# UCL-CCS/Nbed

Measured on AMD Instinct MI355X. Metric: embedded_scf_cycles_per_sec, higher is better.
Workload: dtype f64

## Files before the change

### nbed_amd/csrc/elementwise.hip

```cpp
#include "nbx_common.h"
#include "jk_m4_layout.h"
#include "jk_packed.h"
#include "jk_s4_layout.h"

namespace {

constexpr int TILE = 32;
constexpr int DENS_MAX_NOCC = 64;

__global__ void final_reduce_kernel(const double* __restrict__ partial, int nblocks, int nout,
                                    double* __restrict__ out, int sqrt_from, const int* __restrict__ tail = nullptr,
                                    int tail_n = 0) {
    __shared__ double red[17];
    if ((int)threadIdx.x < tail_n) out[nout + threadIdx.x] = (double)tail[threadIdx.x];
    for (int o = 0; o < nout; ++o) {
        double t = 0.0;
        for (int b = threadIdx.x; b < nblocks; b += blockDim.x) t += partial[(int64_t)b * nout + o];
        t = nbx_block_sum(t, red);
        if (threadIdx.x == 0) out[o] = (o >= sqrt_from) ? sqrt(t) : t;
        __syncthreads();
    }
}

__device__ __forceinline__ void load_tile(const double* __restrict__ M, int N, int r0, int c0,
                                          double (*lds)[TILE + 1]) {
    for (int r = threadIdx.y; r < TILE; r += blockDim.y) {
        const int gr = r0 + r, gc = c0 + threadIdx.x;
        lds[r][threadIdx.x] = (gr < N && gc < N) ? M[(int64_t)gr * N + gc] : 0.0;
    }
}

__global__ void trace_prod_kernel(const double* __restrict__ A, const double* __restrict__ B, int N,
                                  double* __restrict__ partial) {
    __shared__ double bt[TILE][TILE + 1];
    __shared__ double red[17];
    const int b = blockIdx.z;
    const int64_t n2 = (int64_t)N * N;
    A += b * n2;
    B += b * n2;
    const int i0 = blockIdx.y * TILE, j0 = blockIdx.x * TILE;
    load_tile(B, N, j0, i0, bt);
    __syncthreads();
    double acc = 0.0;
    for (int r = threadIdx.y; r < TILE; r += blockDim.y) {
        const int gi = i0 + r, gj = j0 + threadIdx.x;
        if (gi < N && gj < N) acc = fma(A[(int64_t)gi * N + gj], bt[threadIdx.x][r], acc);
    }
    const int tid = threadIdx.y * blockDim.x + threadIdx.x;
    double v = nbx_wave_sum(acc);
    if ((tid & 63) == 0) red[tid >> 6] = v;
    __syncthreads();
    if (tid == 0) {
        double t = 0.0;
        for (int w = 0; w < (int)(blockDim.x * blockDim.y) / 64; ++w) t += red[w];
        const int nblk = gridDim.x * gridDim.y;
        partial[(int64_t)b * nblk + blockIdx.y * gridDim.x + blockIdx.x] = t;
    }
}

__global__ void fock_uhf_kernel(const double* __restrict__ h, int h3d, const double* __restrict__ vemb,
                                const double* __restrict__ jk, double* __restrict__ fock,
                                double* __restrict__ vhf, int64_t n2) {
    const int64_t i = (int64_t)blockIdx.x * blockDim.x + threadIdx.x;
    if (i >= n2) return;
    const double j = jk[i];
#pragma unroll
    for (int x = 0; x < 2; ++x) {
        const double v = j - jk[(1 + x) * n2 + i];
        double f = h[h3d ? x * n2 + i : i] + v;
        if (vemb) f += vemb[x * n2 + i];
        fock[x * n2 + i] = f;
        if (vhf) vhf[x * n2 + i] = v;
    }
}

typedef double ew_v4f64 __attribute__((ext_vector_type(4)));
__global__ __launch_bounds__(64) void huzinaga_fused_kernel(const double* __restrict__ F,
                                                            const double* __restrict__ DS, int N, double kappa,
                                                            double* __restrict__ hz, double* __restrict__ fock_out) {
    __shared__ double t2[16][17], hv[16][17];
    const int ti = blockIdx.y, tj = blockIdx.x;
    if (tj > ti) return;
    const int64_t n2 = (int64_t)N * N;
    F += blockIdx.z * n2;
    DS += blockIdx.z * n2;
    hz += blockIdx.z * n2;
    if (fock_out != nullptr) fock_out += blockIdx.z * n2;
    const int lane = threadIdx.x, fr = lane & 15, fk = lane >> 4;
    const int ri = ti * 16 + fr, rj = tj * 16 + fr;
    const bool oki = ri < N, okj = rj < N;
    const double* fi = F + (int64_t)(oki ? ri : 0) * N;
    const double* fj = F + (int64_t)(okj ? rj : 0) * N;
    const double* dsj = DS + (okj ? rj : 0);
    const double* dsi = DS + (oki ? ri : 0);
    ew_v4f64 acc1 = {0.0, 0.0, 0.0, 0.0}, acc2 = {0.0, 0.0, 0.0, 0.0};
    const bool diag = ti == tj;
    constexpr int HZ_STEPS = 20;
    for (int k0 = 0; k0 < N; k0 += 4 * HZ_STEPS) {
        double a1[HZ_STEPS], b1[HZ_STEPS], a2[HZ_STEPS], b2[HZ_STEPS];
#pragma unroll
        for (int j = 0; j < HZ_STEPS; ++j) {
            const int k = k0 + 4 * j + fk;
            const bool in = k < N;
            a1[j] = (in && oki) ? fi[k] : 0.0;
            b1[j] = (in && okj) ? dsj[(int64_t)k * N] : 0.0;
            a2[j] = (in && okj && !diag) ? fj[k] : 0.0;
            b2[j] = (in && oki && !diag) ? dsi[(int64_t)k * N] : 0.0;
        }
#pragma unroll
        for (int j = 0; j < HZ_STEPS; ++j) {
            if (k0 + 4 * j < N) {
                acc1 = __builtin_amdgcn_mfma_f64_16x16x4f64(a1[j], b1[j], acc1, 0, 0, 0);
                if (!diag) acc2 = __builtin_amdgcn_mfma_f64_16x16x4f64(a2[j], b2[j], acc2, 0, 0, 0);
            }
        }
    }
    if (diag) acc2 = acc1;
#pragma unroll
    for (int r = 0; r < 4; ++r) t2[fk + 4 * r][fr] = acc2[r];
    __syncthreads();
    double val[4];
#pragma unroll
    for (int r = 0; r < 4; ++r) {
        val[r] = -kappa * (acc1[r] + t2[fr][fk + 4 * r]);
        hv[fk + 4 * r][fr] = val[r];
    }
    __syncthreads();
#pragma unroll
    for (int r = 0; r < 4; ++r) {
        const int row = ti * 16 + fk + 4 * r, col = tj * 16 + fr;
        if (row < N && col < N) {
            const int64_t o = (int64_t)row * N + col;
            hz[o] = val[r];
            if (fock_out != nullptr) fock_out[o] = F[o] + val[r];
        }
        if (!diag) {
            const int mrow = tj * 16 + fk + 4 * r, mcol = ti * 16 + fr;
            if (mrow < N && mcol < N) {
                const int64_t o = (int64_t)mrow * N + mcol;
                const double v = hv[fr][fk + 4 * r];
                hz[o] = v;
                if (fock_out != nullptr) fock_out[o] = F[o] + v;
            }
        }
    }
}

__global__ void huzinaga_sym_kernel(const double* __restrict__ fds, int N, double kappa,
                                    double* __restrict__ hz, double* __restrict__ fock) {
    __shared__ double t[TILE][TILE + 1];
    const int b = blockIdx.z;
    const int64_t n2 = (int64_t)N * N;
    fds += b * n2;
    hz += b * n2;
    if (fock) fock += b * n2;
    const int i0 = blockIdx.y * TILE, j0 = blockIdx.x * TILE;
    load_tile(fds, N, j0, i0, t);
    __syncthreads();
    for (int r = threadIdx.y; r < TILE; r += blockDim.y) {
        const int gi = i0 + r, gj = j0 + threadIdx.x;
        if (gi < N && gj < N) {
            const int64_t o = (int64_t)gi * N + gj;
            const double v = -kappa * (fds[o] + t[threadIdx.x][r]);
            hz[o] = v;
            if (fock) fock[o] += v;
        }
    }
}

__global__ void antisym_kernel(const double* __restrict__ a, int N, double* __restrict__ out) {
    __shared__ double t[TILE][TILE + 1];
    const int b = blockIdx.z;
    const int64_t n2 = (int64_t)N * N;
    a += b * n2;
    out += b * n2;
    const int i0 = blockIdx.y * TILE, j0 = blockIdx.x * TILE;
    load_tile(a, N, j0, i0, t);
    __syncthreads();
    for (int r = threadIdx.y; r < TILE; r += blockDim.y) {
        const int gi = i0 + r, gj = j0 + threadIdx.x;
        if (gi < N && gj < N) {
            const int64_t o = (int64_t)gi * N + gj;
            out[o] = t[threadIdx.x][r] - a[o];
        }
    }
}

template <int T, bool DENS = false>
__global__ void huz_scalars_kernel(const double* __restrict__ h, int h3d, const double* __restrict__ vemb,
                                   const double* __restrict__ vhf, const double* __restrict__ hz,
                                   const double* __restrict__ dm, const double* __restrict__ dm_old, int N,
                                   double* __restrict__ partial, double* __restrict__ out_final = nullptr,
                                   const int* __restrict__ tail = nullptr, int tail_n = 0,
                                   int* __restrict__ counter = nullptr, double* __restrict__ dts = nullptr,
                                   int s4_nb_ = 0, int s4_lpt_ = 0, int dts_m4 = 0,
                                   const double* __restrict__ dtail = nullptr, int dtail_n = 0,
                                   const double* __restrict__ cmo = nullptr, int nocc_a = 0, int nocc_b = 0,
                                   double* __restrict__ dm_w = nullptr) {
    __shared__ double dt[2][T][T + 1];
    __shared__ double red[4][16];
    __shared__ int last;
    const int64_t n2 = (int64_t)N * N;
    const int i0 = blockIdx.y * T, j0 = blockIdx.x * T;
    const int tid = threadIdx.y * blockDim.x + threadIdx.x;
    const int nthr = blockDim.x * blockDim.y, nwave = nthr / 64;
    constexpr int R = T / 8;
    double out[4] = {0.0, 0.0, 0.0, 0.0};
    double dsum[R], tsum[R];
    double ham[2][R], dv[2][R], dold[2][R];
    constexpr int DSTEPS = DENS_MAX_NOCC / 4;
    double ca[DENS ? DSTEPS : 1], cb[DENS ? DSTEPS : 1];
    if (DENS) {
        const int x = tid >> 6, lane = tid & 63, fr = lane & 15, fk = lane >> 4;
        const int K = x == 0 ? nocc_a : nocc_b;
        const int ra = i0 + fr, rb = j0 + fr;
        const double* pa = cmo + x * n2 + (int64_t)(ra < N ? ra : 0) * N;
        const double* pb = cmo + x * n2 + (int64_t)(rb < N ? rb : 0) * N;
#pragma unroll
        for (int j = 0; j < DSTEPS; ++j) {
            const int k = 4 * j + fk;
            ca[j] = (k < K && ra < N) ? pa[k] : 0.0;
            cb[j] = (k < K && rb < N) ? pb[k] : 0.0;
        }
    }
#pragma unroll
    for (int x = 0; x < 2; ++x)
#pragma unroll
        for (int k = 0; k < R; ++k) {
            const int r = threadIdx.y + 8 * k;
            const int gr = j0 + r, gc = i0 + threadIdx.x;
            if (!DENS) dt[x][r][threadIdx.x] = (gr < N && gc < N) ? dm[x * n2 + (int64_t)gr * N + gc] : 0.0;
            const int gi = i0 + r, gj = j0 + threadIdx.x;
            const bool in = gi < N && gj < N;
            const int64_t o = in ? (int64_t)gi * N + gj : 0;
            double hm = h[h3d ? x * n2 + o : o] + 0.5 * vhf[x * n2 + o];
            if (hz) hm += hz[x * n2 + o];
            if (vemb) hm += vemb[x * n2 + o];
            ham[x][k] = in ? hm : 0.0;
            if (!DENS) dv[x][k] = in ? dm[x * n2 + o] : 0.0;
            dold[x][k] = in ? dm_old[x * n2 + o] : 0.0;
        }
    if (DENS) {
        const int x = tid >> 6, lane = tid & 63, fr = lane & 15, fk = lane >> 4;
        const int K = x == 0 ? nocc_a : nocc_b;
        ew_v4f64 acc = {0.0, 0.0, 0.0, 0.0};
#pragma unroll
        for (int j = 0; j < DSTEPS; ++j)
            if (4 * j < K) acc = __builtin_amdgcn_mfma_f64_16x16x4f64(ca[j], cb[j], acc, 0, 0, 0);
#pragma unroll
        for (int r = 0; r < 4; ++r) {
            const int row = fk + 4 * r;
            dt[x][row][fr] = acc[r];
            if (i0 + row < N && j0 + fr < N) dm_w[x * n2 + (int64_t)(i0 + row) * N + j0 + fr] = acc[r];
        }
    }
    __syncthreads();
    if (DENS) {
#pragma unroll
        for (int x = 0; x < 2; ++x)
#pragma unroll
            for (int k = 0; k < R; ++k) dv[x][k] = dt[x][threadIdx.y + 8 * k][threadIdx.x];
    }
#pragma unroll
    for (int k = 0; k < R; ++k) dsum[k] = tsum[k] = 0.0;
#pragma unroll
    for (int x = 0; x < 2; ++x)
#pragma unroll
        for (int k = 0; k < R; ++k) {
            const int r = threadIdx.y + 8 * k;
            const double t = DENS ? dv[x][k] : dt[x][threadIdx.x][r];
            out[x] = fma(ham[x][k], t, out[x]);
            const double dd = dv[x][k] - dold[x][k];
            out[2 + x] = fma(dd, dd, out[2 + x]);
            dsum[k] += dv[x][k];
            tsum[k] += t;
        }
#pragma unroll
    for (int k = 0; k < 4; ++k) {
        const double v = nbx_wave_sum_dpp(out[k]);
        if ((tid & 63) == 0) red[k][tid >> 6] = v;
    }
    __syncthreads();
    if (tid < 4) {
        double t = 0.0;
        for (int w = 0; w < nwave; ++w) t += red[tid][w];
        partial[(int64_t)(blockIdx.y * gridDim.x + blockIdx.x) * 4 + tid] = t;
    }
    auto store_dts = [&]() {
        if (dts != nullptr && i0 >= j0 && dts_m4) {
    #pragma unroll
            for (int k = 0; k < R; ++k) {
                const int gi = i0 + threadIdx.y + 8 * k, gj = j0 + threadIdx.x;
                if (gi < N && gj <= gi) dts[m4_weight_index_rt(s4_nb_, s4_lpt_, dts_m4 >> 8, dts_m4 & 255, gi, gj)] = gi == gj ? dsum[k] : dsum[k] + tsum[k];
            }
        } else if (dts != nullptr && i0 >= j0) {
            const S4Geom g = s4_geom(N, s4_nb_);
    #pragma unroll
            for (int k = 0; k < R; ++k) {
                const int gi = i0 + threadIdx.y + 8 * k, gj = j0 + threadIdx.x;
                if (gi < N && gj <= gi) dts[s4_dts_index(g, s4_lpt_, gi, gj)] = gi == gj ? dsum[k] : dsum[k] + tsum[k];
            }
        }
    };
    if (out_final == nullptr) {
        store_dts();
        return;
    }
    const int nblocks = gridDim.x * gridDim.y;
    __threadfence();
    __syncthreads();
    if (tid == 0) {
        const int prev = __hip_atomic_fetch_add(counter, 1, __ATOMIC_ACQ_REL, __HIP_MEMORY_SCOPE_AGENT);
        last = prev == nblocks - 1;
        if (last) __hip_atomic_store(counter, 0, __ATOMIC_RELAXED, __HIP_MEMORY_SCOPE_AGENT);
    }
    __syncthreads();
    if (!last) {
        store_dts();
        return;
    }
    __threadfence();
    if (tid < tail_n) out_final[4 + tid] = (double)tail[tid];
    if (tid < dtail_n) out_final[4 + tail_n + tid] = dtail[tid];
    double t4[4] = {0.0, 0.0, 0.0, 0.0};
    for (int b = tid; b < nblocks; b += nthr)
#pragma unroll
        for (int o = 0; o < 4; ++o)
            t4[o] += __hip_atomic_load(partial + (int64_t)b * 4 + o, __ATOMIC_RELAXED, __HIP_MEMORY_SCOPE_AGENT);
    __syncthreads();
#pragma unroll
    for (int o = 0; o < 4; ++o) {
        const double v = nbx_wave_sum_dpp(t4[o]);
        if ((tid & 63) == 0) red[o][tid >> 6] = v;
    }
    __syncthreads();
    if (tid < 4) {
        double tot = 0.0;
        for (int w = 0; w < nwave; ++w) tot += red[tid][w];
        out_final[tid] = (tid >= 2) ? sqrt(tot) : tot;
    }
    __syncthreads();
    if (tid == 0) {
        __threadfence_system();
        __hip_atomic_store(out_final + 4 + tail_n + dtail_n, 1.0, __ATOMIC_RELEASE, __HIP_MEMORY_SCOPE_SYSTEM);
    }
    store_dts();
}

__global__ void axpby_kernel(int64_t n, double a, const double* __restrict__ x, double b, double* __restrict__ y) {
    for (int64_t i = (int64_t)blockIdx.x * blockDim.x + threadIdx.x; i < n; i += (int64_t)gridDim.x * blockDim.x)
        y[i] = (b == 0.0) ? a * x[i] : fma(a, x[i], b * y[i]);
}

constexpr int MAX_LINCOMB = 16;
struct Coefs {
    double c[MAX_LINCOMB];
};

__global__ void lincomb_kernel(int64_t n, int nvec, Coefs cf, const double* __restrict__ vecs, int64_t stride,
                               double* __restrict__ out) {
    for (int64_t i = (int64_t)blockIdx.x * blockDim.x + threadIdx.x; i < n; i += (int64_t)gridDim.x * blockDim.x) {
        double t = 0.0;
        for (int k = 0; k < nvec; ++k) t = fma(cf.c[k], vecs[k * stride + i], t);
        out[i] = t;
    }
}

__global__ void dots_kernel(int64_t n, int nvec, const double* __restrict__ x, const double* __restrict__ vecs,
                            int64_t stride, double* __restrict__ partial) {
    __shared__ double red[17];
    for (int k = 0; k < nvec; ++k) {
        double t = 0.0;
        for (int64_t i = (int64_t)blockIdx.x * blockDim.x + threadIdx.x; i < n; i += (int64_t)gridDim.x * blockDim.x)
            t = fma(x[i], vecs[k * stride + i], t);
        t = nbx_block_sum(t, red);
        if (threadIdx.x == 0) partial[(int64_t)blockIdx.x * nvec + k] = t;
        __syncthreads();
    }
}

constexpr int DIIS_MAX_SPACE = 16;
constexpr int DIIS_M = DIIS_MAX_SPACE + 1;
constexpr int DIIS_SLOTS = ((DIIS_M + 1) * (DIIS_M + 1) + 63) / 64;
constexpr int DIIS_STATE_HALF = 68;
constexpr int DIIS_STATE_DOUBLES = 2 * DIIS_STATE_HALF;
constexpr long long DIIS_STATE_MAGIC = 0x4e42585f44494953ll;

__global__ __launch_bounds__(256) void diis_push_kernel(int64_t n, int nd, int slot, const double* __restrict__ x,
                                                        const double* __restrict__ xprev,
                                                        const double* __restrict__ err, double* __restrict__ xs,
                                                        double* __restrict__ es, double* __restrict__ partial,
                                                        double* __restrict__ state, int anti_n = 0) {
    __shared__ double red[4][DIIS_MAX_SPACE];
    if (blockIdx.x == 0 && threadIdx.x < DIIS_STATE_HALF) state[threadIdx.x] = state[DIIS_STATE_HALF + threadIdx.x];
    double acc[DIIS_MAX_SPACE];
#pragma unroll
    for (int k = 0; k < DIIS_MAX_SPACE; ++k) acc[k] = 0.0;
    for (int64_t i = (int64_t)blockIdx.x * blockDim.x + threadIdx.x; i < n; i += (int64_t)gridDim.x * blockDim.x) {
        const double xv = x[i];
        double e;
        if (anti_n > 0) {
            const int64_t a2 = (int64_t)anti_n * anti_n, bb = i / a2, rc = i - bb * a2;
            const int64_t r = rc / anti_n, c = rc - r * anti_n;
            e = err[bb * a2 + c * anti_n + r] - err[i];
        } else {
            e = (err != nullptr) ? err[i] : xv - xprev[i];
        }
        xs[(int64_t)slot * n + i] = xv;
        es[(int64_t)slot * n + i] = e;
#pragma unroll
        for (int k = 0; k < DIIS_MAX_SPACE; ++k)
            if (k < nd) acc[k] = fma(e, (k == slot) ? e : es[(int64_t)k * n + i], acc[k]);
    }
#pragma unroll
    for (int k = 0; k < DIIS_MAX_SPACE; ++k) {
        if (k < nd) {
            const double t = nbx_wave_sum_dpp(acc[k]);
            if ((threadIdx.x & 63) == 0) red[threadIdx.x >> 6][k] = t;
        }
    }
    __syncthreads();
    if ((int)threadIdx.x < nd)
        partial[(int64_t)blockIdx.x * nd + threadIdx.x] =
            ((red[0][threadIdx.x] + red[1][threadIdx.x]) + red[2][threadIdx.x]) + red[3][threadIdx.x];
}

__device__ __forceinline__ void diis_jacobi_reg8(double& a, double& v, int m, double fro, int lane) {
    const int r = lane >> 3, c = lane & 7;
    for (int sweep = 0; sweep < 40; ++sweep) {
        double off = (r < c) ? a * a : 0.0;
        off = nbx_wave_sum(off);
        if (off <= 1e-31 * fro) break;
        double mind = (r == c && r < m) ? fabs(a) : 1.0e300;
#pragma unroll
        for (int o = 32; o > 0; o >>= 1) mind = fmin(mind, __shfl_xor(mind, o));
        if (mind - sqrt(2.0 * off) > 1.0e-14) break;
        for (int step = 0; step < 7; ++step) {
            auto mate = [&](int k) {
                if (k == 7) return step;
                if (k == step) return 7;
                int x = 2 * step - k;
                x += x < 0 ? 7 : 0;
                x -= x >= 7 ? 7 : 0;
                return x;
            };
            const int mc = mate(c), mr = mate(r);
// ... 357 lines not shown
    As[lane] = acc;
    __syncthreads();
    double row_c = 0.0, row_r = 0.0;
#pragma unroll
    for (int g = 0; g < 8; ++g) {
        row_c += As[8 * g + c];
        row_r += As[8 * g + r];
    }
    __syncthreads();
    double a = new_row ? row_c : (new_col ? row_r : hold);
    if (blockIdx.x == 0 && (new_row || new_col)) H[(int64_t)r * ldh + c] = a;
    A0[r][c] = a;
    if (lane == 0) lu_failed = 0;
    double v = (r == c) ? 1.0 : 0.0;
    if (warm) {
        Vs[lane] = v_prev;
        __syncthreads();
        double gram = 0.0;
#pragma unroll
        for (int k = 0; k < 8; ++k) gram = fma(Vs[8 * k + r], Vs[8 * k + c], gram);
        Ts[lane] = gram;
        __syncthreads();
        double vg = 0.0;
#pragma unroll
        for (int k = 0; k < 8; ++k) vg = fma(Vs[8 * r + k], Ts[8 * k + c], vg);
        v = 1.5 * v_prev - 0.5 * vg;
        __syncthreads();
        Vs[lane] = v;
        As[lane] = a;
        __syncthreads();
        double hv = 0.0;
#pragma unroll
        for (int k = 0; k < 8; ++k) hv = fma(As[8 * r + k], Vs[8 * k + c], hv);
        Ts[lane] = hv;
        __syncthreads();
        double vhv = 0.0;
#pragma unroll
        for (int k = 0; k < 8; ++k) vhv = fma(Vs[8 * k + r], Ts[8 * k + c], vhv);
        __syncthreads();
        Ts[lane] = vhv;
        __syncthreads();
        a = 0.5 * (vhv + Ts[8 * c + r]);
        __syncthreads();
    }
    const double fro = nbx_wave_sum_dpp(a * a);
    diis_jacobi8(a, v, m, fro, lane, As, Vs);
    As[lane] = a;
    Vs[lane] = v;
    if (blockIdx.x == 0) {
        state[DIIS_STATE_HALF + lane] = v;
        if (lane == 0) state[DIIS_STATE_HALF + 64] = __longlong_as_double(DIIS_STATE_MAGIC);
        if (lane == 1) state[DIIS_STATE_HALF + 65] = (double)m;
    }
    __syncthreads();
    const bool singular = __any(r == c && r < m && fabs(a) < 1e-14);
    if (!singular) {
        if (lane < m) rhs_s[lane] = (lane == 0) ? 1.0 : 0.0;
        __syncthreads();
        for (int k = 0; k < m; ++k) {
            double best = (lane >= k && lane < m) ? fabs(A0[lane][k]) : -1.0;
            int piv = lane;
#pragma unroll
            for (int o = 4; o > 0; o >>= 1) {
                const double ob = __shfl_xor(best, o);
                const int op = __shfl_xor(piv, o);
                if (ob > best || (ob == best && op < piv)) {
                    best = ob;
                    piv = op;
                }
            }
            best = nbx_readlane_f64(best, 0);
            piv = __builtin_amdgcn_readlane(piv, 0);
            if (best == 0.0) {
                if (lane == 0) lu_failed = 1;
                break;
            }
            if (piv != k) {
                if (lane < m) {
                    const double tmp = A0[k][lane];
                    A0[k][lane] = A0[piv][lane];
                    A0[piv][lane] = tmp;
                }
                if (lane == 0) {
                    const double tmp = rhs_s[k];
                    rhs_s[k] = rhs_s[piv];
                    rhs_s[piv] = tmp;
                }
            }
            __syncthreads();
            const double inv = 1.0 / A0[k][k];
            const bool below = r > k && r < m, right = c > k && c < m;
            double upd = 0.0, rupd = 0.0;
            if (below && right) upd = A0[r][c] - (A0[r][k] * inv) * A0[k][c];
            if (below && c == 0) rupd = rhs_s[r] - (A0[r][k] * inv) * rhs_s[k];
            __syncthreads();
            if (below && right) A0[r][c] = upd;
            if (below && c == 0) rhs_s[r] = rupd;
            __syncthreads();
        }
        __syncthreads();
        if (!lu_failed) {
            for (int i = m - 1; i >= 0; --i) {
                const double t = nbx_wave_sum_dpp((lane > i && lane < m) ? A0[i][lane] * c_out[lane] : 0.0);
                if (lane == 0) c_out[i] = (rhs_s[i] - t) / A0[i][i];
                __syncthreads();
            }
        }
        __syncthreads();
    }
    if (singular || lu_failed) {
        const double w = As[9 * c], v0 = Vs[c];
        const bool keep = c < m && (!singular || fabs(w) > 1e-14);
        const double t = nbx_sum8_dpp(keep ? v * (1.0 / w) * v0 : 0.0);
        if (c == 0 && r < m) c_out[r] = t;
        __syncthreads();
    }
    if (blockIdx.x == 0 && lane >= 1 && lane < m) coef[lane - 1] = c_out[lane];
    double cf[DIIS8_MAX_ND];
#pragma unroll
    for (int k = 0; k < DIIS8_MAX_ND; ++k) cf[k] = (k < nd) ? c_out[k + 1] : 0.0;
#pragma unroll
    for (int j = 0; j < DIIS8_PER_LANE; ++j) {
        const int64_t i = i0 + 64 * j;
        if (i < n) {
            double t = 0.0;
#pragma unroll
            for (int k = 0; k < DIIS8_MAX_ND; ++k)
                if (k < nd) t = fma(cf[k], xv[j][k], t);
            out[i] = t;
        }
    }
}

__global__ void lincomb_dev_kernel(int64_t n, int nvec, const double* __restrict__ coef,
                                   const double* __restrict__ vecs, int64_t stride, double* __restrict__ out) {
    for (int64_t i = (int64_t)blockIdx.x * blockDim.x + threadIdx.x; i < n; i += (int64_t)gridDim.x * blockDim.x) {
        double t = 0.0;
        for (int k = 0; k < nvec; ++k) t = fma(coef[k], vecs[k * stride + i], t);
        out[i] = t;
    }
}

__global__ void transpose_kernel(const double* __restrict__ A, double* __restrict__ B, int64_t rows, int64_t cols) {
    __shared__ double t[TILE][TILE + 1];
    const int64_t b = blockIdx.z;
    A += b * rows * cols;
    B += b * rows * cols;
    const int64_t r0 = (int64_t)blockIdx.y * TILE, c0 = (int64_t)blockIdx.x * TILE;
    for (int r = threadIdx.y; r < TILE; r += blockDim.y) {
        const int64_t gr = r0 + r, gc = c0 + threadIdx.x;
        if (gr < rows && gc < cols) t[r][threadIdx.x] = A[gr * cols + gc];
    }
    __syncthreads();
    for (int c = threadIdx.y; c < TILE; c += blockDim.y) {
        const int64_t gc = c0 + c, gr = r0 + threadIdx.x;
        if (gr < rows && gc < cols) B[gc * rows + gr] = t[threadIdx.x][c];
    }
}

__global__ void vo_sumsq_kernel(const double* __restrict__ fmo, int N, int nocc_a, int nocc_b,
                                double* __restrict__ partial) {
    __shared__ double red[17];
    const int x = blockIdx.y;
    const int nocc = x == 0 ? nocc_a : nocc_b;
    const int nvir = N - nocc;
    const int64_t total = (int64_t)nvir * nocc;
    double t = 0.0;
    for (int64_t e = (int64_t)blockIdx.x * blockDim.x + threadIdx.x; e < total; e += (int64_t)gridDim.x * blockDim.x) {
        const int a = nocc + (int)(e / nocc), i = (int)(e % nocc);
        const double v = fmo[((int64_t)x * N + a) * N + i];
        t = fma(v, v, t);
    }
    t = nbx_block_sum(t, red);
    if (threadIdx.x == 0) partial[(int64_t)blockIdx.x * 2 + x] = t;
}

__global__ void scale_cols_kernel(int64_t rows, int64_t cols, const double* __restrict__ s, double* __restrict__ a) {
    const int64_t b = blockIdx.y;
    const int64_t i = (int64_t)blockIdx.x * blockDim.x + threadIdx.x;
    if (i >= rows * cols) return;
    a[b * rows * cols + i] *= s[b * cols + (i % cols)];
}

__global__ void spinorb_h2_kernel(int n, const double* __restrict__ tb, double tol, double scale,
                                  double* __restrict__ h2, int64_t idx0, int64_t count) {
    const int64_t nq = 2 * (int64_t)n;
    const int64_t n4 = (int64_t)n * n * n * n;
    for (int64_t off = (int64_t)blockIdx.x * blockDim.x + threadIdx.x; off < count;
         off += (int64_t)gridDim.x * blockDim.x) {
        const int64_t idx = idx0 + off;
        const int64_t S = idx % nq;
        int64_t t = idx / nq;
        const int64_t R = t % nq;
        t /= nq;
        const int64_t Q = t % nq;
        const int64_t P = t / nq;
        const int sp = (int)(P & 1), sq = (int)(Q & 1), sr = (int)(R & 1), ss = (int)(S & 1);
        int blk = -1;
        if (sp == sq && sq == sr && sr == ss) blk = sp;
        else if (sp == 0 && sq == 1 && sr == 1 && ss == 0) blk = 2;
        else if (sp == 1 && sq == 0 && sr == 0 && ss == 1) blk = 3;
        double v = 0.0;
        if (blk >= 0) {
            const int64_t p = P >> 1, q = Q >> 1, r = R >> 1, s = S >> 1;
            v = tb[blk * n4 + ((p * n + q) * n + r) * n + s];
            if (fabs(v) < tol) v = 0.0;
            v *= scale;
        }
        h2[off] = v;
    }
}

__global__ void threshold_scale_kernel(int64_t n, double tol, double scale, double* __restrict__ x) {
    for (int64_t i = (int64_t)blockIdx.x * blockDim.x + threadIdx.x; i < n; i += (int64_t)gridDim.x * blockDim.x) {
        const double v = x[i];
        x[i] = (fabs(v) < tol ? 0.0 : v) * scale;
    }
}

__global__ void spinorb_h1_kernel(int n, const double* __restrict__ ob, double tol, double* __restrict__ h1) {
    const int nq = 2 * n;
    const int idx = blockIdx.x * blockDim.x + threadIdx.x;
    if (idx >= nq * nq) return;
    const int P = idx / nq, Q = idx % nq;
    double v = 0.0;
    if ((P & 1) == (Q & 1)) {
        v = ob[(int64_t)(P & 1) * n * n + (int64_t)(P >> 1) * n + (Q >> 1)];
        if (fabs(v) < tol) v = 0.0;
    }
    h1[idx] = v;
}

inline unsigned grid1d(int64_t n, int block, int64_t cap = 65536) {
    int64_t g = nbx_cdiv(n, block);
    if (g > cap) g = cap;
    if (g < 1) g = 1;
    return (unsigned)g;
}

int finish_reduction(nbx_ctx* ctx, int nblocks, int nout, double* h_out) {
    hipLaunchKernelGGL(final_reduce_kernel, dim3(1), dim3(256), 0, ctx->stream, ctx->d_scratch, nblocks, nout,
                       ctx->d_scratch + NBX_SCRATCH_DOUBLES - 64, nout);
    NBX_LAUNCH_CHECK();
    NBX_HIP(hipMemcpyAsync(ctx->h_pinned, ctx->d_scratch + NBX_SCRATCH_DOUBLES - 64, nout * sizeof(double),
                           hipMemcpyDeviceToHost, ctx->stream));
    NBX_HIP(hipStreamSynchronize(ctx->stream));
    for (int i = 0; i < nout; ++i) h_out[i] = ctx->h_pinned[i];
    return NBX_OK;
}

inline bool scalars_tiles_fit(int64_t nao, int tile) {
    const int64_t g = nbx_cdiv(nao, tile);
    return g * g * 4 <= NBX_SCRATCH_DOUBLES - 64;
}
inline int scalars_route(int64_t nao) {
    if (nao <= 0) return NBX_CYCLE_SCALARS_REFUSED;
    if (scalars_tiles_fit(nao, 16)) return NBX_CYCLE_SCALARS_T16;
    return scalars_tiles_fit(nao, TILE) ? NBX_CYCLE_SCALARS_T32 : NBX_CYCLE_SCALARS_REFUSED;
}
inline bool density_scalars_fused(int64_t nao, int64_t nocc_a, int64_t nocc_b) {
    return scalars_route(nao) == NBX_CYCLE_SCALARS_T16 && nocc_a > 0 && nocc_b > 0 && nocc_a <= DENS_MAX_NOCC &&
           nocc_b <= DENS_MAX_NOCC;
}
inline int diis_route(int64_t n, int64_t nd) {
    if (n <= 0 || nd < 1 || nd > DIIS_MAX_SPACE) return NBX_DIIS_REFUSED;
    return (nd <= DIIS8_MAX_ND && nbx_cdiv(n, 64 * DIIS8_PER_LANE) <= 65535) ? NBX_DIIS_FUSED : NBX_DIIS_GENERAL;
}
inline int vo_sumsq_route(int64_t nao, int64_t nocc_a, int64_t nocc_b) {
    if (nao <= 0 || nocc_a < 0 || nocc_a > nao || nocc_b < 0 || nocc_b > nao) return NBX_VO_SUMSQ_REFUSED;
    const int64_t na = (nao - nocc_a) * nocc_a, nb = (nao - nocc_b) * nocc_b;
    return (na > nb ? na : nb) <= 16384 ? NBX_VO_SUMSQ_ONE_WG : NBX_VO_SUMSQ_32_WG;
}

}

extern "C" {

int nbx_fock_uhf(nbx_ctx* ctx, int64_t nao, const double* d_hcore, int hcore_ndim, const double* d_vemb,
                 const double* d_jk, double* d_fock, double* d_vhf) {
    NBX_CHECK_ARG(ctx && d_hcore && d_jk && d_fock && nao > 0);
    NBX_CHECK_ARG(hcore_ndim == 2 || hcore_ndim == 3);
    const int64_t n2 = nao * nao;
    hipLaunchKernelGGL(fock_uhf_kernel, dim3((unsigned)nbx_cdiv(n2, 256)), dim3(256), 0, ctx->stream, d_hcore,
                       hcore_ndim == 3 ? 1 : 0, d_vemb, d_jk, d_fock, d_vhf, n2);
    NBX_LAUNCH_CHECK();
    return NBX_OK;
}

int nbx_huzinaga_sym(nbx_ctx* ctx, int64_t nao, int64_t batch, const double* d_fds, double kappa, double* d_hz,
                     double* d_fock_io) {
    NBX_CHECK_ARG(ctx && d_fds && d_hz && nao > 0 && batch > 0 && batch < 65536);
    const unsigned g = (unsigned)nbx_cdiv(nao, TILE);
    hipLaunchKernelGGL(huzinaga_sym_kernel, dim3(g, g, (unsigned)batch), dim3(TILE, 8), 0, ctx->stream, d_fds,
                       (int)nao, kappa, d_hz, d_fock_io);
    NBX_LAUNCH_CHECK();
    return NBX_OK;
}

int nbx_huzinaga_fused(nbx_ctx* ctx, int64_t nao, int64_t batch, const double* d_f, const double* d_ds, double kappa,
                       double* d_hz, double* d_fock_out) {
    NBX_CHECK_ARG(ctx && d_f && d_ds && d_hz && nao > 0 && batch > 0 && batch < 65536);
    NBX_CHECK_ARG(d_fock_out != d_f);
    const unsigned g = (unsigned)nbx_cdiv(nao, 16);
    hipLaunchKernelGGL(huzinaga_fused_kernel, dim3(g, g, (unsigned)batch), dim3(64), 0, ctx->stream, d_f, d_ds,
                       (int)nao, kappa, d_hz, d_fock_out);
    NBX_LAUNCH_CHECK();
    return NBX_OK;
}

int nbx_trace_prod(nbx_ctx* ctx, int64_t nao, int64_t batch, const double* d_a, const double* d_b,
                   double* h_out) {
    NBX_CHECK_ARG(ctx && d_a && d_b && h_out && nao > 0 && batch > 0);
    const int64_t g = nbx_cdiv(nao, TILE);
    NBX_CHECK_ARG(g * g <= NBX_SCRATCH_DOUBLES - 64 && batch <= 64);
    for (int64_t b = 0; b < batch; ++b) {
        hipLaunchKernelGGL(trace_prod_kernel, dim3((unsigned)g, (unsigned)g, 1), dim3(TILE, 8), 0, ctx->stream,
                           d_a + b * nao * nao, d_b + b * nao * nao, (int)nao, ctx->d_scratch);
        NBX_LAUNCH_CHECK();
        const int rc = finish_reduction(ctx, (int)(g * g), 1, h_out + b);
        if (rc != NBX_OK) return rc;
    }
    return NBX_OK;
}

int nbx_huz_cycle_scalars(nbx_ctx* ctx, int64_t nao, const double* d_hcore, int hcore_ndim,
                          const double* d_vemb, const double* d_vhf, const double* d_hz, const double* d_dm,
                          const double* d_dm_old, double* h_out) {
    NBX_CHECK_ARG(ctx && d_hcore && d_vhf && d_hz && d_dm && d_dm_old && h_out && nao > 0);
    NBX_CHECK_ARG(hcore_ndim == 2 || hcore_ndim == 3);
    const int64_t g = nbx_cdiv(nao, TILE);
    NBX_CHECK_ARG(scalars_tiles_fit(nao, TILE));
    hipLaunchKernelGGL(huz_scalars_kernel<TILE>, dim3((unsigned)g, (unsigned)g), dim3(TILE, 8), 0, ctx->stream, d_hcore,
                       hcore_ndim == 3 ? 1 : 0, d_vemb, d_vhf, d_hz, d_dm, d_dm_old, (int)nao, ctx->d_scratch);
    NBX_LAUNCH_CHECK();
    const int rc = finish_reduction(ctx, (int)(g * g), 4, h_out);
    if (rc != NBX_OK) return rc;
    h_out[2] = sqrt(h_out[2]);
    h_out[3] = sqrt(h_out[3]);
    return NBX_OK;
}

int nbx_huz_cycle_scalars_dev(nbx_ctx* ctx, int64_t nao, const double* d_hcore, int hcore_ndim,
                              const double* d_vemb, const double* d_vhf, const double* d_hz, const double* d_dm,
                              const double* d_dm_old, double* d_out, const int* d_tail, int64_t tail_n) {
    return nbx_huz_cycle_scalars_dts(ctx, nao, d_hcore, hcore_ndim, d_vemb, d_vhf, d_hz, d_dm, d_dm_old, d_out, d_tail,
                                     tail_n, nullptr);
}

int nbx_huz_cycle_scalars_dts(nbx_ctx* ctx, int64_t nao, const double* d_hcore, int hcore_ndim,
                              const double* d_vemb, const double* d_vhf, const double* d_hz, const double* d_dm,
                              const double* d_dm_old, double* d_out, const int* d_tail, int64_t tail_n,
                              double* d_dts) {
    NBX_CHECK_ARG(d_hz != nullptr);
    return nbx_cycle_scalars_launch(ctx, nao, d_hcore, hcore_ndim, d_vemb, d_vhf, d_hz, d_dm, d_dm_old, d_out, d_tail,
                                    tail_n, d_dts, nullptr, 0);
}

}

int nbx_cycle_scalars_launch(nbx_ctx* ctx, int64_t nao, const double* d_hcore, int hcore_ndim, const double* d_vemb,
                             const double* d_vhf, const double* d_hz, const double* d_dm, const double* d_dm_old,
                             double* d_out, const int* d_tail, int64_t tail_n, double* d_dts, const double* d_dtail,
                             int64_t dtail_n) {
    NBX_CHECK_ARG(ctx && d_hcore && d_vhf && d_dm && d_dm_old && d_out && nao > 0);
    int nb4 = 0, lpt4 = 0, m4 = 0;
    NBX_CHECK_ARG(d_dts == nullptr || nbx_jk_dts_layout(nao, &nb4, &lpt4, &m4) > 0);
    NBX_CHECK_ARG(tail_n >= 0 && tail_n <= 64 && (tail_n == 0 || d_tail != nullptr));
    NBX_CHECK_ARG(dtail_n >= 0 && dtail_n <= 64 && (dtail_n == 0 || d_dtail != nullptr));
    NBX_CHECK_ARG(hcore_ndim == 2 || hcore_ndim == 3);
    const int route = scalars_route(nao);
    NBX_CHECK_ARG(route != NBX_CYCLE_SCALARS_REFUSED);
    const bool fine = route == NBX_CYCLE_SCALARS_T16;
    const int64_t g = nbx_cdiv(nao, fine ? 16 : TILE);
    if (fine)
        hipLaunchKernelGGL(huz_scalars_kernel<16>, dim3((unsigned)g, (unsigned)g), dim3(16, 8), 0, ctx->stream, d_hcore,
                           hcore_ndim == 3 ? 1 : 0, d_vemb, d_vhf, d_hz, d_dm, d_dm_old, (int)nao, ctx->d_scratch,
                           d_out, d_tail, (int)tail_n, ctx->d_counters + NBX_COUNTERS - 1, d_dts, nb4, lpt4, m4, d_dtail,
                           (int)dtail_n);
    else
        hipLaunchKernelGGL(huz_scalars_kernel<TILE>, dim3((unsigned)g, (unsigned)g), dim3(TILE, 8), 0, ctx->stream,
                           d_hcore, hcore_ndim == 3 ? 1 : 0, d_vemb, d_vhf, d_hz, d_dm, d_dm_old, (int)nao,
                           ctx->d_scratch, d_out, d_tail, (int)tail_n, ctx->d_counters + NBX_COUNTERS - 1, d_dts, nb4,
                           lpt4, m4, d_dtail, (int)dtail_n);
    NBX_LAUNCH_CHECK();
    return NBX_OK;
}

int nbx_density_scalars_launch(nbx_ctx* ctx, int64_t nao, const double* d_hcore, int hcore_ndim, const double* d_vemb,
                               const double* d_vhf, const double* d_hz, const double* d_c, int64_t nocc_a, int64_t nocc_b,
                               double* d_dm_out, const double* d_dm_old, double* d_out, const int* d_tail, int64_t tail_n,
                               double* d_dts) {
    NBX_CHECK_ARG(ctx && d_hcore && d_vhf && d_c && d_dm_out && d_dm_old && d_out && nao > 0);
    if (!density_scalars_fused(nao, nocc_a, nocc_b)) return NBX_E_UNSUPPORTED;
    int nb4 = 0, lpt4 = 0, m4 = 0;
    NBX_CHECK_ARG(d_dts == nullptr || nbx_jk_dts_layout(nao, &nb4, &lpt4, &m4) > 0);
    NBX_CHECK_ARG(tail_n >= 0 && tail_n <= 64 && (tail_n == 0 || d_tail != nullptr));
    NBX_CHECK_ARG(hcore_ndim == 2 || hcore_ndim == 3);
    const int64_t g = nbx_cdiv(nao, 16);
    hipLaunchKernelGGL((huz_scalars_kernel<16, true>), dim3((unsigned)g, (unsigned)g), dim3(16, 8), 0, ctx->stream, d_hcore,
                       hcore_ndim == 3 ? 1 : 0, d_vemb, d_vhf, d_hz, d_dm_out, d_dm_old, (int)nao, ctx->d_scratch, d_out,
                       d_tail, (int)tail_n, ctx->d_counters + NBX_COUNTERS - 1, d_dts, nb4, lpt4, m4, nullptr, 0, d_c,
                       (int)nocc_a, (int)nocc_b, d_dm_out);
    NBX_LAUNCH_CHECK();
    return NBX_OK;
}

int nbx_antisym(nbx_ctx* ctx, int64_t nao, int64_t batch, const double* d_a, double* d_out) {
    NBX_CHECK_ARG(ctx && d_a && d_out && d_a != d_out && nao > 0 && batch > 0 && batch < 65536);
    const unsigned g = (unsigned)nbx_cdiv(nao, TILE);
    hipLaunchKernelGGL(antisym_kernel, dim3(g, g, (unsigned)batch), dim3(TILE, 8), 0, ctx->stream, d_a, (int)nao, d_out);
    NBX_LAUNCH_CHECK();
    return NBX_OK;
}

extern "C" {

size_t nbx_diis_coef_doubles(int64_t space) { return space > 0 ? (size_t)(space + DIIS_STATE_DOUBLES) : 0; }

int nbx_diis_update(nbx_ctx* ctx, int64_t n, int64_t space, int64_t slot, int64_t nd, const double* d_x,
                    double* d_xprev, double* d_xs, double* d_es, double* d_h, double* d_coef) {
    return nbx_diis_update_err(ctx, n, space, slot, nd, d_x, nullptr, d_xprev, d_xs, d_es, d_h, d_coef);
}

int nbx_diis_update_err(nbx_ctx* ctx, int64_t n, int64_t space, int64_t slot, int64_t nd, const double* d_x,
                        const double* d_err, double* d_xprev, double* d_xs, double* d_es, double* d_h,
                        double* d_coef) {
    return nbx_diis_update_anti(ctx, n, space, slot, nd, d_x, d_err, 0, d_xprev, d_xs, d_es, d_h, d_coef);
}

}

int nbx_diis_update_anti(nbx_ctx* ctx, int64_t n, int64_t space, int64_t slot, int64_t nd, const double* d_x,
                         const double* d_err, int64_t anti_n, double* d_xprev, double* d_xs, double* d_es, double* d_h,
                         double* d_coef) {
    NBX_CHECK_ARG(ctx && d_x && d_xprev && d_xs && d_es && d_h && d_coef && n > 0);
    NBX_CHECK_ARG(anti_n == 0 || (d_err != nullptr && anti_n > 0 && n % (anti_n * anti_n) == 0));
    NBX_CHECK_ARG(space >= 1 && space <= DIIS_MAX_SPACE && slot >= 0 && slot < space && nd >= 1 && nd <= space &&
                  slot < nd);
    const unsigned blocks = grid1d(n, 256, 128);
    NBX_CHECK_ARG((int64_t)blocks * nd <= NBX_SCRATCH_DOUBLES - 64);
    hipLaunchKernelGGL(diis_push_kernel, dim3(blocks), dim3(256), 0, ctx->stream, n, (int)nd, (int)slot, d_x,
                       d_xprev, d_err, d_xs, d_es, ctx->d_scratch, d_coef + space, (int)anti_n);
    NBX_LAUNCH_CHECK();
    if (diis_route(n, nd) == NBX_DIIS_FUSED) {
        hipLaunchKernelGGL(diis_solve8_lincomb_kernel, dim3((unsigned)nbx_cdiv(n, 64 * DIIS8_PER_LANE)), dim3(64), 0,
                           ctx->stream, ctx->d_scratch, (int)blocks, (int)nd, (int)slot, d_h, (int)(space + 1), d_coef,
                           d_coef + space, n, d_xs, n, d_xprev);
        NBX_LAUNCH_CHECK();
        return NBX_OK;
    }
    hipLaunchKernelGGL(diis_solve_kernel, dim3(1), dim3(64), 0, ctx->stream, ctx->d_scratch, (int)blocks, (int)nd,
                       (int)slot, d_h, (int)(space + 1), d_coef);
    NBX_LAUNCH_CHECK();
    hipLaunchKernelGGL(lincomb_dev_kernel, dim3(grid1d(n, 256)), dim3(256), 0, ctx->stream, n, (int)nd, d_coef, d_xs,
                       n, d_xprev);
    NBX_LAUNCH_CHECK();
    return NBX_OK;
}

extern "C" {

int nbx_vo_sumsq(nbx_ctx* ctx, int64_t nao, const double* d_fmo, int64_t nocc_a, int64_t nocc_b, double* d_out) {
    NBX_CHECK_ARG(ctx && d_fmo && d_out && nao > 0 && nocc_a >= 0 && nocc_a <= nao && nocc_b >= 0 && nocc_b <= nao);
    if (vo_sumsq_route(nao, nocc_a, nocc_b) == NBX_VO_SUMSQ_ONE_WG) {
        hipLaunchKernelGGL(vo_sumsq_kernel, dim3(1, 2), dim3(256), 0, ctx->stream, d_fmo, (int)nao, (int)nocc_a, (int)nocc_b,
                           d_out);
        NBX_LAUNCH_CHECK();
        return NBX_OK;
    }
    const int blocks = 32;
    hipLaunchKernelGGL(vo_sumsq_kernel, dim3(blocks, 2), dim3(256), 0, ctx->stream, d_fmo, (int)nao, (int)nocc_a,
                       (int)nocc_b, ctx->d_scratch);
    NBX_LAUNCH_CHECK();
    hipLaunchKernelGGL(final_reduce_kernel, dim3(1), dim3(256), 0, ctx->stream, ctx->d_scratch, blocks, 2, d_out, 2);
    NBX_LAUNCH_CHECK();
    return NBX_OK;
}

int nbx_cycle_scalars_route(int64_t nao, int64_t nocc_a, int64_t nocc_b) {
    if (nocc_a >= 0 && nocc_b >= 0 && density_scalars_fused(nao, nocc_a, nocc_b)) return NBX_CYCLE_SCALARS_T16_DENS;
    return scalars_route(nao);
}

int nbx_diis_route(int64_t n, int64_t nd) { return diis_route(n, nd); }

int nbx_vo_sumsq_route(int64_t nao, int64_t nocc_a, int64_t nocc_b) { return vo_sumsq_route(nao, nocc_a, nocc_b); }

int nbx_axpby(nbx_ctx* ctx, int64_t n, double a, const double* d_x, double b, double* d_y) {
    NBX_CHECK_ARG(ctx && n >= 0);
    if (n == 0) return NBX_OK;
    NBX_CHECK_ARG(d_x && d_y);
    hipLaunchKernelGGL(axpby_kernel, dim3(grid1d(n, 256)), dim3(256), 0, ctx->stream, n, a, d_x, b, d_y);
    NBX_LAUNCH_CHECK();
    return NBX_OK;
}

int nbx_lincomb(nbx_ctx* ctx, int64_t n, int64_t nvec, const double* h_coef, const double* d_vecs,
                int64_t stride, double* d_out) {
    NBX_CHECK_ARG(ctx && n >= 0 && nvec > 0 && nvec <= MAX_LINCOMB && h_coef && d_vecs && d_out);
    if (n == 0) return NBX_OK;
    Coefs cf;
    for (int k = 0; k < MAX_LINCOMB; ++k) cf.c[k] = k < nvec ? h_coef[k] : 0.0;
    hipLaunchKernelGGL(lincomb_kernel, dim3(grid1d(n, 256)), dim3(256), 0, ctx->stream, n, (int)nvec, cf, d_vecs,
                       stride, d_out);
    NBX_LAUNCH_CHECK();
    return NBX_OK;
}

int nbx_dots(nbx_ctx* ctx, int64_t n, int64_t nvec, const double* d_x, const double* d_vecs, int64_t stride,
             double* h_out) {
    NBX_CHECK_ARG(ctx && n > 0 && nvec > 0 && nvec <= MAX_LINCOMB && d_x && d_vecs && h_out);
    const unsigned blocks = grid1d(n, 256, 128);
    hipLaunchKernelGGL(dots_kernel, dim3(blocks), dim3(256), 0, ctx->stream, n, (int)nvec, d_x, d_vecs, stride,
                       ctx->d_scratch);
    NBX_LAUNCH_CHECK();
    return finish_reduction(ctx, (int)blocks, (int)nvec, h_out);
}

int nbx_transpose(nbx_ctx* ctx, int64_t rows, int64_t cols, int64_t batch, const double* d_a, double* d_b) {
    NBX_CHECK_ARG(ctx && rows >= 0 && cols >= 0 && batch >= 0);
    if (rows == 0 || cols == 0 || batch == 0) return NBX_OK;
    NBX_CHECK_ARG(d_a && d_b && d_a != d_b);
    const int64_t gy = nbx_cdiv(rows, TILE), gx = nbx_cdiv(cols, TILE);
    if (gy > 65535) {
        nbx_set_error("nbx_transpose: more than 65535*32 rows per matrix is unsupported");
        return NBX_E_UNSUPPORTED;
    }
    for (int64_t b0 = 0; b0 < batch; b0 += 65535) {
        const int64_t nb = (batch - b0) < 65535 ? (batch - b0) : 65535;
        hipLaunchKernelGGL(transpose_kernel, dim3((unsigned)gx, (unsigned)gy, (unsigned)nb), dim3(TILE, 8), 0,
                           ctx->stream, d_a + b0 * rows * cols, d_b + b0 * rows * cols, rows, cols);
        NBX_LAUNCH_CHECK();
    }
    return NBX_OK;
}

int nbx_scale_cols(nbx_ctx* ctx, int64_t rows, int64_t cols, int64_t batch, const double* d_s, double* d_a) {
    NBX_CHECK_ARG(ctx && rows > 0 && cols > 0 && batch > 0 && batch < 65536 && d_s && d_a);
    hipLaunchKernelGGL(scale_cols_kernel, dim3((unsigned)nbx_cdiv(rows * cols, 256), (unsigned)batch), dim3(256), 0,
                       ctx->stream, rows, cols, d_s, d_a);
    NBX_LAUNCH_CHECK();
    return NBX_OK;
}

int nbx_chem_to_phys(nbx_ctx* ctx, int64_t n1, int64_t n2, int64_t n3, int64_t n4, const double* d_in,
                     double* d_out) {
    return nbx_transpose(ctx, n2, n3 * n4, n1, d_in, d_out);
}

int nbx_spinorb_scatter(nbx_ctx* ctx, int64_t n, const double* d_one_body, const double* d_two_body, double tol,
                        double h2_scale, double* d_h1, double* d_h2) {
    NBX_CHECK_ARG(ctx && n > 0 && n < 1024 && d_one_body && d_two_body && d_h1 && d_h2);
    const int64_t nq = 2 * n;
    hipLaunchKernelGGL(spinorb_h1_kernel, dim3((unsigned)nbx_cdiv(nq * nq, 256)), dim3(256), 0, ctx->stream, (int)n,
                       d_one_body, tol, d_h1);
    NBX_LAUNCH_CHECK();
    const int64_t total = nq * nq * nq * nq;
    hipLaunchKernelGGL(spinorb_h2_kernel, dim3(grid1d(total, 256, 8192)), dim3(256), 0, ctx->stream, (int)n,
                       d_two_body, tol, h2_scale, d_h2, (int64_t)0, total);
    NBX_LAUNCH_CHECK();
    return NBX_OK;
}

int nbx_spinorb_scatter_h1(nbx_ctx* ctx, int64_t n, const double* d_one_body, double tol, double* d_h1) {
    NBX_CHECK_ARG(ctx && n > 0 && n < 1024 && d_one_body && d_h1);
    const int64_t nq = 2 * n;
    hipLaunchKernelGGL(spinorb_h1_kernel, dim3((unsigned)nbx_cdiv(nq * nq, 256)), dim3(256), 0, ctx->stream, (int)n,
                       d_one_body, tol, d_h1);
    NBX_LAUNCH_CHECK();
    return NBX_OK;
}

int nbx_spinorb_scatter_range(nbx_ctx* ctx, int64_t n, const double* d_two_body, double tol, double h2_scale,
                              int64_t idx0, int64_t count, double* d_h2_part) {
    NBX_CHECK_ARG(ctx && n > 0 && n < 1024 && d_two_body && idx0 >= 0 && count >= 0);
    const int64_t nq = 2 * n;
    NBX_CHECK_ARG(idx0 + count <= nq * nq * nq * nq);
    if (count == 0) return NBX_OK;
    NBX_CHECK_ARG(d_h2_part != nullptr);
    hipLaunchKernelGGL(spinorb_h2_kernel, dim3(grid1d(count, 256, 8192)), dim3(256), 0, ctx->stream, (int)n,
                       d_two_body, tol, h2_scale, d_h2_part, idx0, count);
    NBX_LAUNCH_CHECK();
    return NBX_OK;
}


int nbx_threshold_scale(nbx_ctx* ctx, int64_t n, double tol, double scale, double* d_x) {
    NBX_CHECK_ARG(ctx && n >= 0);
    if (n == 0) return NBX_OK;
    NBX_CHECK_ARG(d_x != nullptr);
    hipLaunchKernelGGL(threshold_scale_kernel, dim3(grid1d(n, 256, 8192)), dim3(256), 0, ctx->stream, n, tol, scale, d_x);
    NBX_LAUNCH_CHECK();
    return NBX_OK;
}

}
```

Before: 4442.

## Split Huzinaga fused kernel's two MFMA products across two wavefronts

The Huzinaga fused kernel now launches 128 threads per block, so each of the two wavefronts computes one of the two 16x16 products (F·DS for the tile and its mirror) instead of one wavefront doing both serially. The K-loop unroll depth doubles, loads use clamped indices instead of predicated loads, and the F values needed for the fock output are prefetched before the main loop. This aims to roughly halve the per-block MFMA chain latency and raise memory-level parallelism, at the cost of higher register pressure from the deeper unroll and an idle second wave on diagonal tiles.

```diff
diff --git a/nbed_amd/csrc/elementwise.hip b/nbed_amd/csrc/elementwise.hip
--- a/nbed_amd/csrc/elementwise.hip
+++ b/nbed_amd/csrc/elementwise.hip
@@ -75,9 +75,10 @@
 }
 
 typedef double ew_v4f64 __attribute__((ext_vector_type(4)));
-__global__ __launch_bounds__(64) void huzinaga_fused_kernel(const double* __restrict__ F,
-                                                            const double* __restrict__ DS, int N, double kappa,
-                                                            double* __restrict__ hz, double* __restrict__ fock_out) {
+constexpr int HZ_STEPS = 40;
+__global__ __launch_bounds__(128) void huzinaga_fused_kernel(const double* __restrict__ F,
+                                                             const double* __restrict__ DS, int N, double kappa,
+                                                             double* __restrict__ hz, double* __restrict__ fock_out) {
     __shared__ double t2[16][17], hv[16][17];
     const int ti = blockIdx.y, tj = blockIdx.x;
     if (tj > ti) return;
@@ -86,62 +87,62 @@
     DS += blockIdx.z * n2;
     hz += blockIdx.z * n2;
     if (fock_out != nullptr) fock_out += blockIdx.z * n2;
-    const int lane = threadIdx.x, fr = lane & 15, fk = lane >> 4;
-    const int ri = ti * 16 + fr, rj = tj * 16 + fr;
-    const bool oki = ri < N, okj = rj < N;
-    const double* fi = F + (int64_t)(oki ? ri : 0) * N;
-    const double* fj = F + (int64_t)(okj ? rj : 0) * N;
-    const double* dsj = DS + (okj ? rj : 0);
-    const double* dsi = DS + (oki ? ri : 0);
-    ew_v4f64 acc1 = {0.0, 0.0, 0.0, 0.0}, acc2 = {0.0, 0.0, 0.0, 0.0};
+    const int wv = threadIdx.x >> 6, lane = threadIdx.x & 63, fr = lane & 15, fk = lane >> 4;
     const bool diag = ti == tj;
-    constexpr int HZ_STEPS = 20;
-    for (int k0 = 0; k0 < N; k0 += 4 * HZ_STEPS) {
-        double a1[HZ_STEPS], b1[HZ_STEPS], a2[HZ_STEPS], b2[HZ_STEPS];
-#pragma unroll
-        for (int j = 0; j < HZ_STEPS; ++j) {
-            const int k = k0 + 4 * j + fk;
-            const bool in = k < N;
-            a1[j] = (in && oki) ? fi[k] : 0.0;
-            b1[j] = (in && okj) ? dsj[(int64_t)k * N] : 0.0;
-            a2[j] = (in && okj && !diag) ? fj[k] : 0.0;
-            b2[j] = (in && oki && !diag) ? dsi[(int64_t)k * N] : 0.0;
-        }
-#pragma unroll
-        for (int j = 0; j < HZ_STEPS; ++j) {
-            if (k0 + 4 * j < N) {
-                acc1 = __builtin_amdgcn_mfma_f64_16x16x4f64(a1[j], b1[j], acc1, 0, 0, 0);
-                if (!diag) acc2 = __builtin_amdgcn_mfma_f64_16x16x4f64(a2[j], b2[j], acc2, 0, 0, 0);
-            }
-        }
-    }
-    if (diag) acc2 = acc1;
-#pragma unroll
-    for (int r = 0; r < 4; ++r) t2[fk + 4 * r][fr] = acc2[r];
-    __syncthreads();
-    double val[4];
+    const bool work = wv == 0 || !diag;
+    const int ta = wv == 0 ? ti : tj, tb = wv == 0 ? tj : ti;
+    const int ra = ta * 16 + fr, cb = tb * 16 + fr;
+    const bool oka = ra < N, okb = cb < N;
+    const double* fa = F + (int64_t)(oka ? ra : 0) * N;
+    const double* db = DS + (okb ? cb : 0);
+    ew_v4f64 acc = {0.0, 0.0, 0.0, 0.0};
+    double fo[4];
+    int64_t oo[4];
+    bool oin[4];
 #pragma unroll
     for (int r = 0; r < 4; ++r) {
-        val[r] = -kappa * (acc1[r] + t2[fr][fk + 4 * r]);
-        hv[fk + 4 * r][fr] = val[r];
+        const int row = ta * 16 + fk + 4 * r, col = tb * 16 + fr;
+        oin[r] = work && row < N && col < N;
+        oo[r] = oin[r] ? (int64_t)row * N + col : 0;
+        fo[r] = fock_out != nullptr ? F[oo[r]] : 0.0;
+    }
+    if (work) {
+        for (int k0 = 0; k0 < N; k0 += 4 * HZ_STEPS) {
+            double a[HZ_STEPS], b[HZ_STEPS];
+#pragma unroll
+            for (int j = 0; j < HZ_STEPS; ++j) {
+                const int k = k0 + 4 * j + fk, kc = k < N ? k : N - 1;
+                a[j] = fa[kc];
+                b[j] = db[(int64_t)kc * N];
+            }
+#pragma unroll
+            for (int j = 0; j < HZ_STEPS; ++j) {
+                const bool in = k0 + 4 * j + fk < N;
+                if (k0 + 4 * j < N)
+                    acc = __builtin_amdgcn_mfma_f64_16x16x4f64((in && oka) ? a[j] : 0.0, (in && okb) ? b[j] : 0.0, acc, 0, 0, 0);
+            }
+        }
+    }
+    if (wv == (diag ? 0 : 1)) {
+#pragma unroll
+        for (int r = 0; r < 4; ++r) t2[fk + 4 * r][fr] = acc[r];
+    }
+    __syncthreads();
+    double val[4] = {0.0, 0.0, 0.0, 0.0};
+    if (wv == 0) {
+#pragma unroll
+        for (int r = 0; r < 4; ++r) {
+            val[r] = -kappa * (acc[r] + t2[fr][fk + 4 * r]);
+            hv[fk + 4 * r][fr] = val[r];
+        }
     }
     __syncthreads();
 #pragma unroll
     for (int r = 0; r < 4; ++r) {
-        const int row = ti * 16 + fk + 4 * r, col = tj * 16 + fr;
-        if (row < N && col < N) {
-            const int64_t o = (int64_t)row * N + col;
-            hz[o] = val[r];
-            if (fock_out != nullptr) fock_out[o] = F[o] + val[r];
-        }
-        if (!diag) {
-            const int mrow = tj * 16 + fk + 4 * r, mcol = ti * 16 + fr;
-            if (mrow < N && mcol < N) {
-                const int64_t o = (int64_t)mrow * N + mcol;
-                const double v = hv[fr][fk + 4 * r];
-                hz[o] = v;
-                if (fock_out != nullptr) fock_out[o] = F[o] + v;
-            }
+        if (oin[r]) {
+            const double v = wv == 0 ? val[r] : hv[fr][fk + 4 * r];
+            hz[oo[r]] = v;
+            if (fock_out != nullptr) fock_out[oo[r]] = fo[r] + v;
         }
     }
 }
@@ -1105,7 +1106,7 @@
     NBX_CHECK_ARG(ctx && d_f && d_ds && d_hz && nao > 0 && batch > 0 && batch < 65536);
     NBX_CHECK_ARG(d_fock_out != d_f);
     const unsigned g = (unsigned)nbx_cdiv(nao, 16);
-    hipLaunchKernelGGL(huzinaga_fused_kernel, dim3(g, g, (unsigned)batch), dim3(64), 0, ctx->stream, d_f, d_ds,
+    hipLaunchKernelGGL(huzinaga_fused_kernel, dim3(g, g, (unsigned)batch), dim3(128), 0, ctx->stream, d_f, d_ds,
                        (int)nao, kappa, d_hz, d_fock_out);
     NBX_LAUNCH_CHECK();
     return NBX_OK;
```

After: 4580, median of 6. 3.1% higher.
